# alexrenz/AdaPM

Measured on AMD Instinct MI355X. Metric: pull_push_ops_per_s, higher is better.
Workload: dtype fp32; 1 GPU; model=kge_complex_dim512, entities=10000000, relations=1000, dim=512, neg_samples=16, global_batch=16384, triples=90000000, parallelism=ps-async-dp1, fused_step=True, warmup_extra_steps=400

## Files before the change

### adapm_amd/csrc/core.cpp

```cpp
#include <torch/extension.h>
#include <ATen/Parallel.h>

#include <algorithm>
#include <atomic>
#include <condition_variable>
#include <cstring>
#include <limits>
#include <deque>
#include <map>
#include <queue>
#include <tuple>
#include <memory>
#include <mutex>
#include <random>
#include <thread>
#include <chrono>
#include <unordered_map>
#include <unordered_set>
#include <cstdio>
#include <vector>

#include "common.h"
#include "kernels.h"
#include "ops.h"
// ... 211 lines not shown
    state_ = torch::zeros({USTREAM_STATE_WORDS},
                          torch::TensorOptions().dtype(torch::kInt64).device(dev_));
  }

  static bool supported(int64_t lo, int64_t hi) {
    if (hi <= lo || lo == std::numeric_limits<int64_t>::min()) return false;
    uint64_t span = (uint64_t)hi - (uint64_t)lo;
    return span >= 2 && span <= 0xFFFFFFFFull;
  }

  void import_state(uint64_t state_hi, uint64_t state_lo, uint64_t inc_hi, uint64_t inc_lo,
                    uint64_t has_uint32, uint64_t uinteger) {
    auto h = torch::empty({USTREAM_STATE_WORDS}, torch::kInt64);
    uint64_t* p = reinterpret_cast<uint64_t*>(h.data_ptr<int64_t>());
    p[0] = state_hi, p[1] = state_lo, p[2] = inc_hi, p[3] = inc_lo;
    p[4] = has_uint32 ? 1 : 0, p[5] = uinteger & 0xFFFFFFFFull;
    ustream_build_table(p);
    std::lock_guard<std::mutex> g(mu_);
    adopt(current_stream(dev_));
    state_.copy_(h);
  }

  std::vector<uint64_t> export_state() {
    torch::Tensor h;
    {
      std::lock_guard<std::mutex> g(mu_);
      adopt(current_stream(dev_));
      h = state_.slice(0, 0, USTREAM_GEN_WORDS).cpu();
    }
    const uint64_t* p = reinterpret_cast<const uint64_t*>(h.data_ptr<int64_t>());
    return std::vector<uint64_t>(p, p + USTREAM_GEN_WORDS);
  }

  torch::Tensor draw(int64_t n, int64_t slack = -1) {
    TORCH_CHECK(n >= 0, "UniformStream.draw: n must be >= 0");
    auto opt = torch::TensorOptions().dtype(torch::kInt64).device(dev_);
    auto out = torch::empty({n}, opt);
    if (n == 0) return out;
    if (slack < 0) {
      double p = (double)thr_ / 4294967296.0;
      double w0 = (double)n / (1.0 - p);
      slack = (int64_t)std::ceil(w0 - (double)n + 8.0 * std::sqrt(w0 * p) / (1.0 - p)) + 16;
    }
    const int64_t words = n + slack;
    std::lock_guard<std::mutex> g(mu_);
    void* st = current_stream(dev_);
    adopt(st);
    auto tmp = torch::empty({ustream_tmp_words(words)}, opt);
    uint64_t* sp = reinterpret_cast<uint64_t*>(state_.data_ptr<int64_t>());
    if (dev_.is_cuda()) {
#ifdef ADAPM_WITH_HIP
      uniform_draw_gpu(sp, lo_, excl_, thr_, n, words, out.data_ptr<int64_t>(),
                       tmp.data_ptr<int64_t>(), st);
#else
      TORCH_CHECK(false, "UniformStream: built without HIP");
#endif
    } else {
      uniform_draw_cpu(sp, lo_, excl_, thr_, n, words, out.data_ptr<int64_t>(),
                       tmp.data_ptr<int64_t>());
    }
    return out;
  }

  int64_t lo() const { return lo_; }
  int64_t hi() const { return hi_; }
  const torch::Device& device() const { return dev_; }

 private:
  void adopt(void* st) {
#ifdef ADAPM_WITH_HIP
    if (dev_.is_cuda() && have_owner_ && st != owner_) hipStreamSynchronize((hipStream_t)owner_);
#endif
    owner_ = st;
    have_owner_ = true;
  }

  int64_t lo_, hi_;
  uint32_t excl_ = 0, thr_ = 0;
  torch::Device dev_;
  torch::Tensor state_;
  std::mutex mu_;
  void* owner_ = nullptr;
  bool have_owner_ = false;
};


// ... 2108 lines not shown
      ChannelState& C = channels_[ch];
      C.rounds++;
      if (globally_idle) {
        if (++C.idle_streak >= 2) C.idle2_events++;
      } else {
        C.idle_streak = 0;
      }
    }
    rounds_cv_.notify_all();
  }

  py::dict debug_pending() {
    py::dict d;
    {
      std::lock_guard<std::mutex> g(tickets_mu_);
      d["tickets"] = tickets_.size();
    }
    py::list outq, respq, rounds;
    for (auto& C : channels_) {
      std::lock_guard<std::mutex> g(C.mu);
      outq.append(C.out_queue.size());
      respq.append(C.responses.size());
      rounds.append(C.rounds.load());
    }
    d["out_queues"] = outq;
    d["responses"] = respq;
    d["rounds"] = rounds;
    return d;
  }


  bool fused_plain_ok(void* st) {
    if (clocks_.size() != 1 || fused_multi_stream_) return false;
    if (!fused_marks_.defined()) {
      if (getenv("ADAPM_FUSED_ATOMIC")) {
        fused_multi_stream_ = true;
        return false;
      }
      fused_marks_ = torch::zeros({rowmark_words(num_keys_)},
                                  torch::TensorOptions().dtype(torch::kInt32).device(dev_));
      if (getenv("ADAPM_FUSED_STATS"))
        fused_shared_stat_ =
            torch::zeros({1}, torch::TensorOptions().dtype(torch::kInt64).device(dev_));
      fused_marks_stream_ = st;
      return true;
    }
    if (st == fused_marks_stream_) return true;
#ifdef ADAPM_WITH_HIP
    hipStreamSynchronize((hipStream_t)fused_marks_stream_);
#endif
    fused_multi_stream_ = true;
    return false;
  }

  void check_fused_identity(const char* name, int64_t D) {
    TORCH_CHECK(world_ == 1, name, " requires a single rank (all keys local)");
    TORCH_CHECK(uniform_len_ == 2 * D, name, ": store rows must be [emb|accum] = 2D");
    TORCH_CHECK(layout_identity_.load(), name, " requires the identity layout");
    TORCH_CHECK(dev_.is_cuda(), name, " is the GPU fast path");
  }

  void count_fused_ops(int64_t keys) {
    stat_pull_keys_ += keys;
    stat_pull_local_ += keys;
    stat_push_keys_ += keys;
    stat_push_local_ += keys;
    stat_pulls_ += 1;
    stat_pushes_ += 1;
  }

  struct StagedKeys {
    torch::Tensor dev;
    std::vector<const int64_t*> ptr;
  };
  StagedKeys stage_keys(const char* name, std::initializer_list<const torch::Tensor*> parts) {
    int64_t total = 0;
    for (auto* t : parts) {
      check_keys(*t);
      total += t->numel();
    }
    auto blob = torch::empty(
        {total}, torch::TensorOptions().dtype(torch::kInt64).pinned_memory(true));
    int64_t* dst = blob.data_ptr<int64_t>();
    const uint64_t lim = (uint64_t)num_keys_;
    uint64_t bad = 0;
    for (auto* t : parts) {
      const int64_t* kp = t->data_ptr<int64_t>();
      const int64_t n = t->numel();
      for (int64_t i = 0; i < n; ++i) {
        int64_t k = kp[i];
        dst[i] = k;
        bad |= ((uint64_t)k >= lim);
      }
      dst += n;
    }
    if (bad)
      for (auto* t : parts) check_key_range(*t);
    StagedKeys sk;
    sk.dev = torch::empty({total}, torch::TensorOptions().dtype(torch::kInt64).device(dev_));
#ifdef ADAPM_WITH_HIP
    auto stream = c10::hip::getCurrentHIPStreamMasqueradingAsCUDA(dev_.index());
    TORCH_CHECK(copy_keys_gpu(sk.dev.data_ptr<int64_t>(), blob.data_ptr<int64_t>(), total,
                              (void*)stream.stream()),
                name, ": the pinned key staging buffer is not visible to the device");
    at::getHostAllocator(at::kCUDA)->record_event(
        blob.data_ptr(), blob.storage().data_ptr().get_context(), stream.unwrap());
#else
    TORCH_CHECK(false, name, ": built without HIP");
#endif
    const int64_t* dp = sk.dev.data_ptr<int64_t>();
    for (auto* t : parts) {
      sk.ptr.push_back(dp);
      dp += t->numel();
    }
    return sk;
  }

  std::tuple<torch::Tensor, torch::Tensor> kge_step_fused_impl(
      const torch::Tensor& keys_s, const torch::Tensor& keys_r, const torch::Tensor& keys_o,
      const torch::Tensor* keys_neg, UniformStream* us, int64_t N, int64_t D, double lr,
      double eps) {
    check_fused_identity("kge_step_fused", D);
    check_step_lanes("kge_step_fused", "D/2", D / 2);
    int64_t B = keys_s.numel();
    TORCH_CHECK(keys_r.numel() == B && keys_o.numel() == B);
    StagedKeys sk;
    torch::Tensor drawn;
    const int64_t* kn;
    if (us) {
      TORCH_CHECK(us->lo() >= 0 && us->hi() <= num_keys_, "kge_step_fused_sampled: stream range [",
                  us->lo(), ", ", us->hi(), ") exceeds the store's ", num_keys_, " keys");
      TORCH_CHECK(us->device() == dev_,
                  "kge_step_fused_sampled: stream is not on the store's device");
      TORCH_CHECK(N >= 0 && B * N > 0, "kge_step_fused_sampled: nothing to draw");
      sk = stage_keys("kge_step_fused", {&keys_s, &keys_r, &keys_o});
      drawn = us->draw(B * N);
      kn = drawn.data_ptr<int64_t>();
    } else {
      TORCH_CHECK(keys_neg->numel() == B * N);
      sk = stage_keys("kge_step_fused", {&keys_s, &keys_r, &keys_o, keys_neg});
      kn = sk.ptr[3];
    }
    const int64_t *ks = sk.ptr[0], *kr = sk.ptr[1], *ko = sk.ptr[2];

    auto loss = torch::empty({B}, torch::TensorOptions().dtype(torch::kFloat32).device(dev_));
    void* st = current_stream(dev_);
    {
      InflightGuard g(this);
      std::unique_lock<std::mutex> mg(fused_mu_);
      if (fused_plain_ok(st)) {
        RowMarkKeys mk{{ks, kr, ko, kn}, {B, B, B, B * N}, 4};
        auto* marks = reinterpret_cast<uint32_t*>(fused_marks_.data_ptr<int32_t>());
        rowmark_set_gpu(marks, mk, st);
        kge_complex_step_fused_gpu(
            slab_.data, mk.keys[0], mk.keys[1], mk.keys[2], mk.keys[3], loss.data_ptr<float>(),
            (int)B, (int)N, (int)D, Slab::padded(uniform_len_), world_, (float)lr, (float)eps,
            st, marks,
            fused_shared_stat_.defined()
                ? reinterpret_cast<unsigned long long*>(fused_shared_stat_.data_ptr<int64_t>())
                : nullptr);
        rowmark_clear_gpu(marks, mk, st);
        stat_fused_plain_ += 1;
      } else {
        mg.unlock();
        kge_complex_step_fused_gpu(slab_.data, ks, kr, ko, kn, loss.data_ptr<float>(), (int)B,
                                   (int)N, (int)D, Slab::padded(uniform_len_), world_, (float)lr,
                                   (float)eps, st);
        stat_fused_atomic_ += 1;
      }
    }
    count_fused_ops(3 * B + B * N);
    return {loss, drawn};
  }

  torch::Tensor kge_step_fused(torch::Tensor keys_s, torch::Tensor keys_r, torch::Tensor keys_o,
                               torch::Tensor keys_neg, int64_t N, int64_t D, double lr,
                               double eps) {
    return std::get<0>(
        kge_step_fused_impl(keys_s, keys_r, keys_o, &keys_neg, nullptr, N, D, lr, eps));
  }

  std::tuple<torch::Tensor, torch::Tensor> kge_step_fused_sampled(
      torch::Tensor keys_s, torch::Tensor keys_r, torch::Tensor keys_o, UniformStream& us,
      int64_t N, int64_t D, double lr, double eps) {
    return kge_step_fused_impl(keys_s, keys_r, keys_o, nullptr, &us, N, D, lr, eps);
  }

  struct FusedResolve {
    std::vector<std::vector<int64_t>> offs;
    std::vector<int64_t> missed;
    int64_t b_hit = 0;
    std::vector<const int64_t*> ptr;
    std::vector<torch::Tensor> dev;
  };

  FusedResolve resolve_fused(const std::vector<std::pair<const int64_t*, int>>& arrs,
                             int64_t B) {
    FusedResolve out;
    const int na = (int)arrs.size();
    constexpr int64_t G = 1024;
    int64_t nchunks = (B + G - 1) / G;
    struct Part {
      std::vector<std::vector<int64_t>> offs;
      std::vector<int64_t> missed;
    };
    std::vector<Part> parts(nchunks);
    pass_pool_.run(nchunks, [&](int64_t c0, int64_t c1) {
      for (int64_t c = c0; c < c1; ++c) {
        Part& P = parts[c];
        P.offs.resize(na);
        int64_t e = std::min(B, (c + 1) * G);
        std::vector<int64_t> tmp;
        for (int64_t b = c * G; b < e; ++b) {
          tmp.clear();
          bool ok = true;
          for (int a = 0; a < na && ok; ++a) {
            const int64_t* kp = arrs[a].first;
            int cnt = arrs[a].second;
// ... 585 lines not shown
  std::atomic<int64_t> t_pass_{0}, t_todev_{0}, t_launch_{0}, t_calls_{0}, t_misc_{0};
  std::atomic<int64_t> t_sy_intents_{0}, t_sy_replicas_{0}, t_sy_build_{0}, t_sy_proc_{0},
      t_sy_apply_{0}, n_sy_deltas_{0}, n_sy_proc_recs_{0}, n_sy_apply_recs_{0};
  bool cpp_timing_ = getenv("ADAPM_CPP_TIMING") != nullptr;
 private:
  std::mutex tickets_mu_;
  std::condition_variable tickets_cv_;
  std::unordered_map<int64_t, std::unique_ptr<Ticket>> tickets_;
  std::unordered_map<int64_t, std::string> failed_tickets_;
  std::string failed_reason_;
  std::atomic<bool> failed_flag_{false};
  std::mutex rounds_mu_;
  std::condition_variable rounds_cv_;

  bool locality_stats_ = false;
  std::vector<std::atomic<uint32_t>> key_accesses_, key_local_;
  std::mutex trace_mu_;
  std::unordered_set<Key> traced_keys_;
  bool trace_all_ = false;
  struct TraceEv { double t; Key k; const char* ev; };
  std::vector<TraceEv> trace_;
  std::chrono::steady_clock::time_point t0_ = std::chrono::steady_clock::now();

  std::atomic<int64_t> hop_hist_[9] = {};
  std::atomic<int64_t> stat_replica_records_{0}, stat_replica_payloads_{0};
  std::atomic<int64_t> stat_pulls_{0}, stat_pushes_{0}, stat_pull_keys_{0}, stat_push_keys_{0},
      stat_pull_local_{0}, stat_push_local_{0}, stat_pull_replica_{0}, stat_push_replica_{0},
      stat_remote_pulls_served_{0}, stat_remote_pushes_served_{0}, stat_relocations_{0},
      stat_relocated_in_{0}, stat_replications_{0}, stat_drops_{0}, stat_forwards_{0},
      stat_dropped_records_{0}, stat_delta_overhops_{0}, stat_bytes_sent_{0},
      stat_bytes_recv_{0}, stat_sampling_checks_{0};

  std::mutex fused_mu_;
  torch::Tensor fused_marks_;
  torch::Tensor fused_shared_stat_;
  void* fused_marks_stream_ = nullptr;
  bool fused_multi_stream_ = false;
  std::atomic<int64_t> stat_fused_plain_{0}, stat_fused_atomic_{0};
};


static float* fp(torch::Tensor& t) { return t.data_ptr<float>(); }
static const float* cfp(const torch::Tensor& t) { return t.data_ptr<float>(); }

static void check_f32(const torch::Tensor& t, const char* name) {
  TORCH_CHECK(t.is_contiguous() && t.scalar_type() == torch::kFloat32, name,
              " must be contiguous float32");
}

void kge_complex_step(torch::Tensor s, torch::Tensor r, torch::Tensor o, torch::Tensor neg,
                      torch::Tensor ds, torch::Tensor dr, torch::Tensor do_, torch::Tensor dneg,
                      torch::Tensor loss, int64_t N, int64_t D, double lr, double eps) {
  for (auto* t : {&s, &r, &o, &neg, &ds, &dr, &do_, &dneg, &loss}) check_f32(*t, "kge tensor");
  int B = (int)loss.numel();
  if (s.is_cuda()) {
    TORCH_CHECK(hip_available(), "kge_complex_step: CUDA tensor but no HIP device");
    check_step_lanes("kge_complex_step", "D/2", D / 2);
    kge_complex_step_gpu(cfp(s), cfp(r), cfp(o), cfp(neg), fp(ds), fp(dr), fp(do_), fp(dneg),
                         fp(loss), B, (int)N, (int)D, (float)lr, (float)eps,
                         current_stream(s.device()));
  } else {
    kge_complex_step_cpu(cfp(s), cfp(r), cfp(o), cfp(neg), fp(ds), fp(dr), fp(do_), fp(dneg),
                         fp(loss), B, (int)N, (int)D, (float)lr, (float)eps);
  }
}

void rescal_step(torch::Tensor s, torch::Tensor r, torch::Tensor o, torch::Tensor neg,
                 torch::Tensor ds, torch::Tensor drl, torch::Tensor do_, torch::Tensor dneg,
                 torch::Tensor loss, int64_t N, int64_t D, double lr, double eps) {
// ... 317 lines not shown
      .def(py::init<int64_t, torch::Tensor, int, int, int, int, std::string, double, int, bool,
                    int64_t, int64_t, double>(),
           py::arg("num_keys"), py::arg("value_lengths"), py::arg("rank"), py::arg("world"),
           py::arg("num_channels"), py::arg("num_workers"), py::arg("device"),
           py::arg("capacity_factor") = 2.0, py::arg("techniques") = 0,
           py::arg("location_caches") = true, py::arg("device_cap_floats") = 0,
           py::arg("host_spill_floats") = 0, py::arg("sync_threshold") = 0.0)
      .def("pull", &Server::pull, py::call_guard<py::gil_scoped_release>())
      .def("push", &Server::push, py::call_guard<py::gil_scoped_release>())
      .def("pull_if_local", &Server::pull_if_local, py::call_guard<py::gil_scoped_release>())
      .def("is_local", &Server::is_local)
      .def("intent", &Server::intent, py::call_guard<py::gil_scoped_release>())
      .def("advance_clock", &Server::advance_clock)
      .def("current_clock", &Server::current_clock)
      .def("worker_clocks", &Server::worker_clocks)
      .def("wait", &Server::wait, py::call_guard<py::gil_scoped_release>())
      .def("wait_all", &Server::wait_all, py::call_guard<py::gil_scoped_release>())
      .def("is_finished", &Server::is_finished)
      .def("round_counts", &Server::round_counts)
      .def("wait_rounds", &Server::wait_rounds, py::call_guard<py::gil_scoped_release>())
      .def("idle_counts", &Server::idle_counts)
      .def("wait_idle", &Server::wait_idle, py::call_guard<py::gil_scoped_release>())
      .def("set_intent_ahead", &Server::set_intent_ahead)
      .def("sync_collect", &Server::sync_collect, py::call_guard<py::gil_scoped_release>())
      .def("sync_process", &Server::sync_process, py::call_guard<py::gil_scoped_release>())
      .def("sync_respond", &Server::sync_respond, py::call_guard<py::gil_scoped_release>())
      .def("sync_apply", &Server::sync_apply, py::call_guard<py::gil_scoped_release>())
      .def("sync_finish", &Server::sync_finish, py::arg("ch"),
           py::arg("globally_idle") = false, py::call_guard<py::gil_scoped_release>())
      .def("fail", &Server::fail, py::call_guard<py::gil_scoped_release>())
      .def("failed_reason", &Server::failed_reason)
      .def("scan_local", &Server::scan_local, py::call_guard<py::gil_scoped_release>())
      .def("kge_step_fused", &Server::kge_step_fused, py::call_guard<py::gil_scoped_release>())
      .def("kge_step_fused_sampled", &Server::kge_step_fused_sampled,
           py::call_guard<py::gil_scoped_release>())
      .def("w2v_step_fused", &Server::w2v_step_fused, py::call_guard<py::gil_scoped_release>())
      .def("mf_step_fused", &Server::mf_step_fused, py::call_guard<py::gil_scoped_release>())
      .def("kge_step_fused_general", &Server::kge_step_fused_general,
           py::call_guard<py::gil_scoped_release>())
      .def("w2v_step_fused_general", &Server::w2v_step_fused_general,
           py::call_guard<py::gil_scoped_release>())
      .def("mf_step_fused_general", &Server::mf_step_fused_general,
           py::call_guard<py::gil_scoped_release>())
      .def("rebalance_spill", &Server::rebalance_spill, py::arg("max_moves") = 4096,
           py::call_guard<py::gil_scoped_release>())
      .def("key_tier", &Server::key_tier)
      .def("get_len", &Server::get_len)
      .def("uniform_len", &Server::uniform_len)
      .def("layout_identity", &Server::layout_identity)
      .def("num_keys", &Server::num_keys)
      .def("rank", &Server::rank)
      .def("world", &Server::world)
      .def("num_channels", &Server::num_channels)
      .def("owner_hint", &Server::owner_hint)
      .def("enable_locality_stats", &Server::enable_locality_stats)
      .def("enable_key_trace", &Server::enable_key_trace)
      .def("debug_key_state", &Server::debug_key_state)
      .def("debug_set_loc_cache", &Server::debug_set_loc_cache)
      .def("debug_pending", &Server::debug_pending)
      .def("dump_locality_stats", &Server::dump_locality_stats)
      .def("dump_traces", &Server::dump_traces)
      .def("stats", &Server::stats)
      .def("debug_flags", &Server::debug_flags);
}
```

### adapm_amd/csrc/kernels.h

```cpp
#pragma once
#include <cstdint>

namespace adapm {

constexpr int STEP_MAX_LANES = 8 * 256;

void kge_complex_step_gpu(const float* s, const float* r, const float* o, const float* neg,
                          float* ds, float* dr, float* do_, float* dneg, float* loss,
                          int B, int N, int D, float lr, float eps, void* stream);
void kge_complex_step_cpu(const float* s, const float* r, const float* o, const float* neg,
                          float* ds, float* dr, float* do_, float* dneg, float* loss,
                          int B, int N, int D, float lr, float eps);

struct RowMarkKeys {
  const int64_t* keys[4];
  int64_t n[4];
  int count;
};
inline int64_t rowmark_words(int64_t rows) { return (rows + 15) / 16; }
void rowmark_set_gpu(uint32_t* marks, const RowMarkKeys& ks, void* stream);
void rowmark_clear_gpu(uint32_t* marks, const RowMarkKeys& ks, void* stream);

void kge_complex_step_fused_gpu(float* slab, const int64_t* keys_s, const int64_t* keys_r,
                                const int64_t* keys_o, const int64_t* keys_neg, float* loss,
                                int B, int N, int D, int32_t plen, int world, float lr,
                                float eps, void* stream, const uint32_t* marks = nullptr,
                                unsigned long long* shared_stat = nullptr);

void kge_complex_step_fused_offs_cpu(float* slab, const int64_t* offs_s, const int64_t* offs_r,
                                     const int64_t* offs_o, const int64_t* offs_neg, float* loss,
                                     int B, int N, int D, float lr, float eps);
void w2v_sgns_step_fused_offs_cpu(float* slab, const int64_t* offs_ctr, const int64_t* offs_ctx,
                                  const int64_t* offs_neg, float* loss, int B, int N, int D,
                                  float lr, float eps);
void mf_update_step_fused_offs_cpu(float* slab, const int64_t* offs_w, const int64_t* offs_h,
                                   const float* x, float* loss, int B, int R, float lr,
                                   float lambda, float eps);

void w2v_sgns_step_fused_gpu(float* slab, const int64_t* keys_ctr, const int64_t* keys_ctx,
                             const int64_t* keys_neg, float* loss, int B, int N, int D,
                             int32_t plen, int world, float lr, float eps, void* stream);

void mf_update_step_fused_gpu(float* slab, const int64_t* keys_w, const int64_t* keys_h,
                              const float* x, float* loss, int B, int R, int32_t plen,
                              int world, float lr, float lambda, float eps, void* stream);

void kge_complex_score_gpu(const float* s, const float* r, const float* cand, float* scores,
                           int B, int E, int D, void* stream);
void kge_complex_score_cpu(const float* s, const float* r, const float* cand, float* scores,
                           int B, int E, int D);

void rescal_step_gpu(const float* s, const float* r, const float* o, const float* neg,
                     float* ds, float* drl, float* do_, float* dneg, float* loss, int B, int N,
                     int D, float lr, float eps, void* stream);
void rescal_step_cpu(const float* s, const float* r, const float* o, const float* neg,
                     float* ds, float* drl, float* do_, float* dneg, float* loss, int B, int N,
                     int D, float lr, float eps);

void w2v_sgns_step_gpu(const float* ctr, const float* ctx, const float* neg, float* dctr,
                       float* dctx, float* dneg, float* loss, int B, int N, int D, float lr,
                       float eps, void* stream);
void w2v_sgns_step_cpu(const float* ctr, const float* ctx, const float* neg, float* dctr,
                       float* dctx, float* dneg, float* loss, int B, int N, int D, float lr,
                       float eps);

void mf_update_step_gpu(const float* w, const float* h, const float* x, float* dw, float* dh,
                        float* loss, int B, int R, float lr, float lambda, float eps,
                        void* stream);
void mf_update_step_cpu(const float* w, const float* h, const float* x, float* dw, float* dh,
                        float* loss, int B, int R, float lr, float lambda, float eps);

void mf_loss_gpu(const float* w, const float* h, const float* x, double* acc2, int B, int R,
                 float lambda, void* stream);
void mf_loss_cpu(const float* w, const float* h, const float* x, float* out2, int B, int R,
                 float lambda);

void alias_draw_gpu(const float* prob, const int32_t* alias, int64_t n, uint64_t seed,
                    int64_t N, int64_t* out, void* stream);
void alias_draw_cpu(const float* prob, const int32_t* alias, int64_t n, uint64_t seed,
                    int64_t N, int64_t* out);

void uniform_draw_gpu(uint64_t* state, int64_t lo, uint32_t excl, uint32_t thr, int64_t n,
                      int64_t words, int64_t* out, int64_t* tmp, void* stream);
void uniform_draw_cpu(uint64_t* state, int64_t lo, uint32_t excl, uint32_t thr, int64_t n,
                      int64_t words, int64_t* out, int64_t* tmp);

bool copy_keys_gpu(int64_t* dst, const int64_t* src_host, int64_t n, void* stream);

}

namespace adapm {


void kge_complex_score_mfma_gpu(const float* s, const float* r, const float* cand,
                                float* scores, float* qbuf, int B, int E, int D, void* stream);

void mfma_grouped_gemm_gpu(const float* S, const float* W, const float* R, float* out,
                           const int* starts, int G, int D, int sstride, int wstride,
                           int64_t rstride, int out_rstride, int64_t ostride, int mode,
                           int total_tiles, void* stream);

void rescal_mid_gpu(const float* U, const float* o, const float* neg, float* do_, float* dneg,
                    float* Wm, float* loss, int B, int N, int D, float lr, float eps,
                    void* stream);

void adagrad_rows_gpu(const float* grad, const float* rows, float* out, int64_t n_rows,
                      int dvals, int gstride, int rstride, float lr, float eps, void* stream);

}
```

### adapm_amd/csrc/kernels_hip.hip

```cpp
#include <hip/hip_runtime.h>
#include <algorithm>
#include <type_traits>

#include "kernels.h"
#include "ustream.h"

namespace adapm {

#define KT 256

static inline unsigned grid_for(int64_t n, int64_t cap = 16384) {
  return (unsigned)std::min(std::max<int64_t>(n, 1), cap);
}

static_assert(STEP_MAX_LANES == 8 * KT, "dispatch_kpt stops at KPT = 8");
template <typename F>
static inline void dispatch_kpt(int lanes, F&& f) {
  if (lanes <= KT) f(std::integral_constant<int, 1>{});
  else if (lanes <= 2 * KT) f(std::integral_constant<int, 2>{});
  else if (lanes <= 4 * KT) f(std::integral_constant<int, 4>{});
  else f(std::integral_constant<int, 8>{});
}

__device__ inline float block_reduce_sum(float v, float* lds) {
// ... 283 lines not shown
                           int B, int E, int D, void* stream) {
  hipLaunchKernelGGL(k_kge_score, dim3(grid_for((int64_t)B * E)), dim3(KT), 0,
                     (hipStream_t)stream, s, r, cand, scores, B, E, D);
}
void w2v_sgns_step_gpu(const float* ctr, const float* ctx, const float* neg, float* dctr,
                       float* dctx, float* dneg, float* loss, int B, int N, int D, float lr,
                       float eps, void* stream) {
  dispatch_kpt(D, [&](auto kpt) {
    hipLaunchKernelGGL(k_w2v_step<decltype(kpt)::value>, dim3(grid_for(B)), dim3(KT), 0,
                       (hipStream_t)stream, ctr, ctx, neg, dctr, dctx, dneg, loss, B, N, D, lr,
                       eps);
  });
}
void mf_update_step_gpu(const float* w, const float* h, const float* x, float* dw, float* dh,
                        float* loss, int B, int R, float lr, float lambda, float eps,
                        void* stream) {
  hipLaunchKernelGGL(k_mf_step, dim3(grid_for(B)), dim3(KT), 0, (hipStream_t)stream, w, h, x, dw,
                     dh, loss, B, R, lr, lambda, eps);
}

}

namespace adapm {
void alias_draw_gpu(const float* prob, const int32_t* alias, int64_t n, uint64_t seed,
                    int64_t N, int64_t* out, void* stream) {
  if (N == 0) return;
  hipLaunchKernelGGL(k_alias_draw, dim3(grid_for((N + 255) / 256, 4096)), dim3(256), 0,
                     (hipStream_t)stream, prob, alias, n, seed, N, out);
}
}

namespace adapm {

static_assert(USTREAM_BLOCK == KT, "one chunk per thread of a KT workgroup");

__device__ inline int64_t block_reduce_i64(int64_t v, int64_t* lds) {
  for (int off = 32; off > 0; off >>= 1) v += __shfl_xor(v, off, 64);
  if ((threadIdx.x & 63) == 0) lds[threadIdx.x >> 6] = v;
  __syncthreads();
  int64_t out = 0;
  for (int i = 0; i < KT / 64; ++i) out += lds[i];
  __syncthreads();
  return out;
}

template <typename T>
__device__ inline T* ustream_block_keys(T* tmp, int64_t nb, int64_t block) {
  return tmp + USTREAM_TMP_COUNTS + nb + block * (KT * USTREAM_CHUNK) + threadIdx.x;
}

__global__ void __launch_bounds__(KT)
k_ustream_gen(const uint64_t* __restrict__ state, UStreamRange r, int64_t words, int64_t chunks,
              int64_t* __restrict__ tmp, int64_t nb) {
  __shared__ int64_t lds[KT / 64];
  const int64_t c = (int64_t)blockIdx.x * KT + threadIdx.x;
  int64_t cnt = 0;
  if (c < chunks)
    cnt = ustream_gen_chunk(state, r, words, c, ustream_block_keys(tmp, nb, blockIdx.x), KT);
  cnt = block_reduce_i64(cnt, lds);
  if (threadIdx.x == 0) {
    tmp[USTREAM_TMP_COUNTS + blockIdx.x] = cnt;
  }
}

__global__ void __launch_bounds__(KT)
k_ustream_compact(uint64_t* __restrict__ state, UStreamRange r, int64_t n, int64_t words,
                  int64_t chunks, const int64_t* __restrict__ tmp, int64_t nb,
                  int64_t* __restrict__ out) {
  __shared__ int64_t lds[KT / 64];
  __shared__ int wave_tot[KT / 64];
  const int64_t* counts = tmp + USTREAM_TMP_COUNTS;
  int64_t part = 0;
  for (int64_t i = threadIdx.x; i < (int64_t)blockIdx.x; i += KT) part += counts[i];
  const int64_t off = block_reduce_i64(part, lds);
  const int64_t c = (int64_t)blockIdx.x * KT + threadIdx.x;
  const bool live = off < n && c < chunks;
  const int64_t* kc = ustream_block_keys(tmp, nb, blockIdx.x);
  int64_t k[USTREAM_CHUNK];
  int cnt = 0;
#pragma unroll
  for (int i = 0; i < USTREAM_CHUNK; ++i) {
    k[i] = live ? kc[i * KT] : USTREAM_REJECTED;
    cnt += (k[i] != USTREAM_REJECTED);
  }
  const int lane = threadIdx.x & 63, wave = threadIdx.x >> 6;
  int incl = cnt;
  for (int d = 1; d < 64; d <<= 1) {
    int y = __shfl_up(incl, d, 64);
    if (lane >= d) incl += y;
  }
  if (lane == 63) wave_tot[wave] = incl;
  __syncthreads();
  int64_t idx = off + incl - cnt;
  for (int i = 0; i < wave; ++i) idx += wave_tot[i];
  int64_t consumed = 0;
#pragma unroll
  for (int i = 0; i < USTREAM_CHUNK; ++i) {
    if (k[i] == USTREAM_REJECTED) continue;
    if (idx < n) {
      out[idx] = k[i];
      if (idx == n - 1) consumed = c * USTREAM_CHUNK + i + 1;
    }
    ++idx;
  }
  if (consumed) {
    ustream_finish(state, r, n, words, n, consumed, out);
  } else if (blockIdx.x == nb - 1 && threadIdx.x == 0) {
    int64_t total = off;
    for (int i = 0; i < KT / 64; ++i) total += wave_tot[i];
    if (total < n) ustream_finish(state, r, n, words, total, 0, out);
  }
}

void uniform_draw_gpu(uint64_t* state, int64_t lo, uint32_t excl, uint32_t thr, int64_t n,
                      int64_t words, int64_t* out, int64_t* tmp, void* stream) {
  if (n <= 0) return;
  const UStreamRange r{lo, excl, thr};
  const int64_t chunks = ustream_chunks(words), nb = ustream_blocks(words);
  auto st = (hipStream_t)stream;
  hipLaunchKernelGGL(k_ustream_gen, dim3((unsigned)nb), dim3(KT), 0, st, state, r, words, chunks,
                     tmp, nb);
  hipLaunchKernelGGL(k_ustream_compact, dim3((unsigned)nb), dim3(KT), 0, st, state, r, n, words,
                     chunks, tmp, nb, out);
}

__global__ void k_copy_keys(int64_t* __restrict__ dst, const int64_t* __restrict__ src,
                            int64_t n) {
  int64_t i = (int64_t)blockIdx.x * KT + threadIdx.x;
  if (i < n) dst[i] = src[i];
}

bool copy_keys_gpu(int64_t* dst, const int64_t* src_host, int64_t n, void* stream) {
  if (n <= 0) return true;
  void* src = nullptr;
  if (hipHostGetDevicePointer(&src, const_cast<int64_t*>(src_host), 0) != hipSuccess || !src) {
    (void)hipGetLastError();
    return false;
  }
  hipLaunchKernelGGL(k_copy_keys, dim3((unsigned)((n + KT - 1) / KT)), dim3(KT), 0,
                     (hipStream_t)stream, dst, static_cast<const int64_t*>(src), n);
  return true;
}
}

namespace adapm {

__global__ void k_rescal_step(const float* __restrict__ s, const float* __restrict__ r,
                              const float* __restrict__ o, const float* __restrict__ neg,
                              float* __restrict__ ds, float* __restrict__ drl,
                              float* __restrict__ do_, float* __restrict__ dneg,
                              float* __restrict__ loss, int B, int N, int D, float lr,
                              float eps) {
  extern __shared__ __attribute__((aligned(16))) float smem[];
  float* Rm = smem;
  float* u = Rm + D * D;
  float* w = u + D;
  float* es = w + D;
  float* red = es + D;
  const int erow = 2 * D;
  const int64_t rrow = 2LL * D * D;

  for (int b = blockIdx.x; b < B; b += gridDim.x) {
    const float* sb = s + (int64_t)b * erow;
    const float* rb = r + (int64_t)b * rrow;
    for (int i = threadIdx.x; i < D * D; i += KT) Rm[i] = rb[i];
    for (int i = threadIdx.x; i < D; i += KT) {
      es[i] = sb[i];
      w[i] = 0.f;
    }
    __syncthreads();
    for (int j = threadIdx.x; j < D; j += KT) {
      float a = 0.f;
      for (int i = 0; i < D; ++i) a += Rm[i * D + j] * es[i];
// ... 24 lines not shown
    float* dsb = ds + (int64_t)b * erow;
    for (int i = threadIdx.x; i < D; i += KT) {
      float a = 0.f;
      for (int k = 0; k < D; ++k) a += Rm[i * D + k] * w[k];
      write_delta(&dsb[i], &dsb[D + i], a, sb[D + i], lr, eps);
    }
    float* drb = drl + (int64_t)b * rrow;
    for (int idx = threadIdx.x; idx < D * D; idx += KT) {
      int i = idx / D, k = idx % D;
      const int64_t acc = (int64_t)D * D + idx;
      write_delta(&drb[idx], &drb[acc], es[i] * w[k], rb[acc], lr, eps);
    }
    __syncthreads();
  }
}

void rescal_step_gpu(const float* s, const float* r, const float* o, const float* neg,
                     float* ds, float* drl, float* do_, float* dneg, float* loss, int B, int N,
                     int D, float lr, float eps, void* stream) {
  size_t smem = (size_t)(D * D + 3 * D + KT / 64) * sizeof(float);
  if (B < 1) return;
  hipLaunchKernelGGL(k_rescal_step, dim3(grid_for(B, 8192)), dim3(KT), smem, (hipStream_t)stream,
                     s, r, o, neg, ds, drl, do_, dneg, loss, B, N, D, lr, eps);
}

}

namespace adapm {

__device__ inline float* row_at(float* slab, int64_t v, int32_t plen, int world) {
  return world ? slab + (v / world) * (int64_t)plen : slab + v;
}

__device__ inline uint32_t* rowmark_word(uint32_t* marks, int64_t row) { return marks + (row >> 4); }
__device__ inline int rowmark_shift(int64_t row) { return 2 * (int)(row & 15); }

__device__ inline int64_t rowmark_key(const RowMarkKeys& ks, int64_t i) {
  int a = 0;
  while (a < ks.count - 1 && i >= ks.n[a]) {
    i -= ks.n[a];
    ++a;
  }
  return ks.keys[a][i];
}

__global__ void k_rowmark_set(uint32_t* __restrict__ marks, RowMarkKeys ks, int64_t total) {
  int64_t i = (int64_t)blockIdx.x * blockDim.x + threadIdx.x;
  if (i >= total) return;
  int64_t row = rowmark_key(ks, i);
  uint32_t bit = 1u << rowmark_shift(row);
  uint32_t old = atomicOr(rowmark_word(marks, row), bit);
  if ((old & bit) && !(old & (bit << 1))) atomicOr(rowmark_word(marks, row), bit << 1);
}

__global__ void k_rowmark_clear(uint32_t* __restrict__ marks, RowMarkKeys ks, int64_t total) {
  int64_t i = (int64_t)blockIdx.x * blockDim.x + threadIdx.x;
  if (i >= total) return;
  *rowmark_word(marks, rowmark_key(ks, i)) = 0u;
}

void rowmark_set_gpu(uint32_t* marks, const RowMarkKeys& ks, void* stream) {
  int64_t total = 0;
  for (int a = 0; a < ks.count; ++a) total += ks.n[a];
  if (total == 0) return;
  hipLaunchKernelGGL(k_rowmark_set, dim3((unsigned)((total + KT - 1) / KT)), dim3(KT), 0,
                     (hipStream_t)stream, marks, ks, total);
}

void rowmark_clear_gpu(uint32_t* marks, const RowMarkKeys& ks, void* stream) {
  int64_t total = 0;
  for (int a = 0; a < ks.count; ++a) total += ks.n[a];
  if (total == 0) return;
  hipLaunchKernelGGL(k_rowmark_clear, dim3((unsigned)((total + KT - 1) / KT)), dim3(KT), 0,
                     (hipStream_t)stream, marks, ks, total);
}

template <bool UNIQ>
__device__ inline bool row_shared(const uint32_t* __restrict__ marks, int64_t key) {
  if (!UNIQ) return true;
  return (marks[key >> 4] >> (rowmark_shift(key) + 1)) & 1u;
}

__device__ inline float plain_add(float a, float delta) {
#pragma clang fp contract(off)
  return a + delta;
}

__device__ inline void slab_adagrad(float* p_emb, float* p_acc, float g, float emb, float acc,
                                    float lr, float eps, bool shared) {
  float d = adagrad_delta(g, acc, lr, eps);
  if (shared) {
    atomicAdd(p_emb, d);
    atomicAdd(p_acc, g * g);
  } else {
    *p_emb = plain_add(emb, d);
    *p_acc = plain_add(acc, g * g);
  }
}

#define SLAB_ADAGRAD_COMPLEX(row, shared, g_re, g_im, emb_re, emb_im, acc_re, acc_im) \
  do {                                                                                \
    float G_re = (acc_re) + (g_re) * (g_re);                                          \
    float G_im = (acc_im) + (g_im) * (g_im);                                          \
    float d_re = -lr * (g_re) * __frsqrt_rn(G_re + eps);                              \
    float d_im = -lr * (g_im) * __frsqrt_rn(G_im + eps);                              \
    if (shared) {                                                                     \
      atomicAdd(&(row)[k], d_re);                                                     \
      atomicAdd(&(row)[dc + k], d_im);                                                \
      atomicAdd(&(row)[D + k], (g_re) * (g_re));                                      \
      atomicAdd(&(row)[D + dc + k], (g_im) * (g_im));                                 \
    } else {                                                                          \
      (row)[k] = plain_add(emb_re, d_re);                                             \
      (row)[dc + k] = plain_add(emb_im, d_im);                                        \
      (row)[D + k] = plain_add(acc_re, (g_re) * (g_re));                              \
      (row)[D + dc + k] = plain_add(acc_im, (g_im) * (g_im));                         \
    }                                                                                 \
  } while (0)

template <int KPT, bool UNIQ>
__global__ void k_kge_step_fused(float* __restrict__ slab, const int64_t* __restrict__ keys_s,
                                 const int64_t* __restrict__ keys_r,
                                 const int64_t* __restrict__ keys_o,
                                 const int64_t* __restrict__ keys_neg, float* __restrict__ loss,
                                 int B, int N, int D, int32_t plen, int world, float lr,
                                 float eps, const uint32_t* __restrict__ marks,
                                 unsigned long long* __restrict__ shared_stat) {
  __shared__ float lds[KT / 64];
  const int dc = D >> 1;
  const int w = UNIQ ? 1 : world;
  for (int b = blockIdx.x; b < B; b += gridDim.x) {
    const int64_t key_s = keys_s[b], key_r = keys_r[b];
    const float* sb = row_at(slab, key_s, plen, w);
    const float* rb = row_at(slab, key_r, plen, w);
    const bool s_shared = row_shared<UNIQ>(marks, key_s);
    const bool r_shared = row_shared<UNIQ>(marks, key_r);
    unsigned n_shared = (unsigned)s_shared + (unsigned)r_shared;

    float s_re[KPT], s_im[KPT], r_re[KPT], r_im[KPT];
    float a_sre[KPT], a_sim[KPT], a_rre[KPT], a_rim[KPT];
    float u_re[KPT], u_im[KPT];
#pragma unroll
    for (int i = 0; i < KPT; ++i) {
      int k = threadIdx.x + i * KT;
      a_sre[i] = a_sim[i] = a_rre[i] = a_rim[i] = 0.f;
      if (k < dc) {
        s_re[i] = sb[k];
        s_im[i] = sb[dc + k];
        r_re[i] = rb[k];
        r_im[i] = rb[dc + k];
        u_re[i] = s_re[i] * r_re[i] - s_im[i] * r_im[i];
        u_im[i] = s_im[i] * r_re[i] + s_re[i] * r_im[i];
      } else {
        s_re[i] = s_im[i] = r_re[i] = r_im[i] = u_re[i] = u_im[i] = 0.f;
      }
    }

    float lsum = 0.f;
    for (int j = 0; j <= N; ++j) {
      int64_t ok = (j == 0) ? keys_o[b] : keys_neg[(int64_t)b * N + (j - 1)];
      float* ob = row_at(slab, ok, plen, w);
      const bool o_shared = row_shared<UNIQ>(marks, ok);
      n_shared += (unsigned)o_shared;
      float y = (j == 0) ? 1.f : -1.f;
      float part = 0.f;
      float o_re[KPT], o_im[KPT], Go_re[KPT], Go_im[KPT];
#pragma unroll
      for (int i = 0; i < KPT; ++i) {
        int k = threadIdx.x + i * KT;
        o_re[i] = k < dc ? ob[k] : 0.f;
        o_im[i] = k < dc ? ob[dc + k] : 0.f;
        Go_re[i] = k < dc ? ob[D + k] : 0.f;
        Go_im[i] = k < dc ? ob[D + dc + k] : 0.f;
        part += u_re[i] * o_re[i] + u_im[i] * o_im[i];
      }
      float psi = block_reduce_sum(part, lds);
      float c = -y * sigmoidf(-y * psi);
      if (threadIdx.x == 0) lsum += softplusf(-y * psi);

#pragma unroll
      for (int i = 0; i < KPT; ++i) {
        int k = threadIdx.x + i * KT;
        if (k >= dc) continue;
        a_sre[i] += c * (r_re[i] * o_re[i] + r_im[i] * o_im[i]);
        a_sim[i] += c * (r_re[i] * o_im[i] - r_im[i] * o_re[i]);
        a_rre[i] += c * (s_re[i] * o_re[i] + s_im[i] * o_im[i]);
        a_rim[i] += c * (s_re[i] * o_im[i] - s_im[i] * o_re[i]);
        float g_re = c * u_re[i];
        float g_im = c * u_im[i];
        SLAB_ADAGRAD_COMPLEX(ob, o_shared, g_re, g_im, o_re[i], o_im[i], Go_re[i], Go_im[i]);
      }
    }
    float* dsb = const_cast<float*>(sb);
    float* drb = const_cast<float*>(rb);
#pragma unroll
    for (int i = 0; i < KPT; ++i) {
      int k = threadIdx.x + i * KT;
      if (k >= dc) continue;
      float Gs_re = sb[D + k], Gs_im = sb[D + dc + k];
      SLAB_ADAGRAD_COMPLEX(dsb, s_shared, a_sre[i], a_sim[i], s_re[i], s_im[i], Gs_re, Gs_im);
      float Gr_re = rb[D + k], Gr_im = rb[D + dc + k];
      SLAB_ADAGRAD_COMPLEX(drb, r_shared, a_rre[i], a_rim[i], r_re[i], r_im[i], Gr_re, Gr_im);
    }
    if (threadIdx.x == 0) {
      loss[b] = lsum;
      if (UNIQ && shared_stat) atomicAdd(shared_stat, (unsigned long long)n_shared);
    }
  }
}

#undef SLAB_ADAGRAD_COMPLEX

void kge_complex_step_fused_gpu(float* slab, const int64_t* keys_s, const int64_t* keys_r,
                                const int64_t* keys_o, const int64_t* keys_neg, float* loss,
                                int B, int N, int D, int32_t plen, int world, float lr,
                                float eps, void* stream, const uint32_t* marks,
                                unsigned long long* shared_stat) {
  if (B < 1) return;
  const bool uniq = marks != nullptr && world == 1;
  if (!uniq) marks = nullptr, shared_stat = nullptr;
  dispatch_kpt(D >> 1, [&](auto kpt) {
    constexpr int KPT = decltype(kpt)::value;
    hipLaunchKernelGGL((uniq ? k_kge_step_fused<KPT, true> : k_kge_step_fused<KPT, false>),
                       dim3(grid_for(B)), dim3(KT), 0, (hipStream_t)stream, slab, keys_s, keys_r,
                       keys_o, keys_neg, loss, B, N, D, plen, world, lr, eps, marks,
                       shared_stat);
  });
}

}

namespace adapm {

template <int KPT>
__global__ void k_w2v_step_fused(float* __restrict__ slab, const int64_t* __restrict__ keys_ctr,
                                 const int64_t* __restrict__ keys_ctx,
                                 const int64_t* __restrict__ keys_neg, float* __restrict__ loss,
                                 int B, int N, int D, int32_t plen, int world, float lr,
                                 float eps) {
  __shared__ float lds[KT / 64];
  for (int b = blockIdx.x; b < B; b += gridDim.x) {
    float* cb = row_at(slab, keys_ctr[b], plen, world);
    float c_emb[KPT], a_c[KPT];
#pragma unroll
    for (int i = 0; i < KPT; ++i) {
      int k = threadIdx.x + i * KT;
      c_emb[i] = k < D ? cb[k] : 0.f;
      a_c[i] = 0.f;
    }
    float lsum = 0.f;
    for (int j = 0; j <= N; ++j) {
      int64_t xk = (j == 0) ? keys_ctx[b] : keys_neg[(int64_t)b * N + (j - 1)];
      float* xb = row_at(slab, xk, plen, world);
      float y = (j == 0) ? 1.f : -1.f;
      float part = 0.f;
      float x_emb[KPT];
#pragma unroll
      for (int i = 0; i < KPT; ++i) {
        int k = threadIdx.x + i * KT;
// ... 68 lines not shown
```

Before: 1.229 billion key-ops/s.

## Replace row-mark bitmap with per-slot owner table claimed during key staging

Duplicate-row detection used to run in separate passes: an atomic set kernel over a packed 2-bit bitmap, then a clear kernel after the step. Now the key copy and uniform-draw compaction kernels write each key's slot index into a per-row owner array (non-atomic, last writer wins). A single resolve kernel then flags both the slots that lost and the winning slot as shared, and the step kernel looks up sharedness by slot index instead of by row. This removes the clear pass and the atomics, and fuses the marking into kernels that already run. In exchange it allocates a full num_keys int32 owner table plus a per-batch shared array, and it relies on the last-writer-wins race to give a consistent winner within each step.

```diff
diff --git a/adapm_amd/csrc/core.cpp b/adapm_amd/csrc/core.cpp
--- a/adapm_amd/csrc/core.cpp
+++ b/adapm_amd/csrc/core.cpp
@@ -267,8 +267,11 @@
     return std::vector<uint64_t>(p, p + USTREAM_GEN_WORDS);
   }
 
-  torch::Tensor draw(int64_t n, int64_t slack = -1) {
+  torch::Tensor draw(int64_t n, int64_t slack = -1) { return draw_owned(n, slack, RowOwners{}, 0); }
+
+  torch::Tensor draw_owned(int64_t n, int64_t slack, RowOwners own, int64_t first) {
     TORCH_CHECK(n >= 0, "UniformStream.draw: n must be >= 0");
+    TORCH_CHECK(!own.owner || dev_.is_cuda(), "UniformStream: row owners need a device stream");
     auto opt = torch::TensorOptions().dtype(torch::kInt64).device(dev_);
     auto out = torch::empty({n}, opt);
     if (n == 0) return out;
@@ -286,7 +289,7 @@
     if (dev_.is_cuda()) {
 #ifdef ADAPM_WITH_HIP
       uniform_draw_gpu(sp, lo_, excl_, thr_, n, words, out.data_ptr<int64_t>(),
-                       tmp.data_ptr<int64_t>(), st);
+                       tmp.data_ptr<int64_t>(), st, own, first);
 #else
       TORCH_CHECK(false, "UniformStream: built without HIP");
 #endif
@@ -2461,22 +2464,22 @@
 
   bool fused_plain_ok(void* st) {
     if (clocks_.size() != 1 || fused_multi_stream_) return false;
-    if (!fused_marks_.defined()) {
+    if (!fused_owner_.defined()) {
       if (getenv("ADAPM_FUSED_ATOMIC")) {
         fused_multi_stream_ = true;
         return false;
       }
-      fused_marks_ = torch::zeros({rowmark_words(num_keys_)},
+      fused_owner_ = torch::zeros({num_keys_},
                                   torch::TensorOptions().dtype(torch::kInt32).device(dev_));
       if (getenv("ADAPM_FUSED_STATS"))
         fused_shared_stat_ =
             torch::zeros({1}, torch::TensorOptions().dtype(torch::kInt64).device(dev_));
-      fused_marks_stream_ = st;
+      fused_owner_stream_ = st;
       return true;
     }
-    if (st == fused_marks_stream_) return true;
+    if (st == fused_owner_stream_) return true;
 #ifdef ADAPM_WITH_HIP
-    hipStreamSynchronize((hipStream_t)fused_marks_stream_);
+    hipStreamSynchronize((hipStream_t)fused_owner_stream_);
 #endif
     fused_multi_stream_ = true;
     return false;
@@ -2502,7 +2505,8 @@
     torch::Tensor dev;
     std::vector<const int64_t*> ptr;
   };
-  StagedKeys stage_keys(const char* name, std::initializer_list<const torch::Tensor*> parts) {
+  StagedKeys stage_keys(const char* name, std::initializer_list<const torch::Tensor*> parts,
+                        RowOwners own = RowOwners{}) {
     int64_t total = 0;
     for (auto* t : parts) {
       check_keys(*t);
@@ -2530,7 +2534,7 @@
 #ifdef ADAPM_WITH_HIP
     auto stream = c10::hip::getCurrentHIPStreamMasqueradingAsCUDA(dev_.index());
     TORCH_CHECK(copy_keys_gpu(sk.dev.data_ptr<int64_t>(), blob.data_ptr<int64_t>(), total,
-                              (void*)stream.stream()),
+                              (void*)stream.stream(), own),
                 name, ": the pinned key staging buffer is not visible to the device");
     at::getHostAllocator(at::kCUDA)->record_event(
         blob.data_ptr(), blob.storage().data_ptr().get_context(), stream.unwrap());
@@ -2547,56 +2551,58 @@
 
   std::tuple<torch::Tensor, torch::Tensor> kge_step_fused_impl(
       const torch::Tensor& keys_s, const torch::Tensor& keys_r, const torch::Tensor& keys_o,
-      const torch::Tensor* keys_neg, UniformStream* us, int64_t N, int64_t D, double lr,
-      double eps) {
+      const torch::Tensor* keys_neg, UniformStream* us, int64_t us_slack, int64_t N, int64_t D,
+      double lr, double eps) {
     check_fused_identity("kge_step_fused", D);
     check_step_lanes("kge_step_fused", "D/2", D / 2);
     int64_t B = keys_s.numel();
     TORCH_CHECK(keys_r.numel() == B && keys_o.numel() == B);
-    StagedKeys sk;
-    torch::Tensor drawn;
-    const int64_t* kn;
     if (us) {
       TORCH_CHECK(us->lo() >= 0 && us->hi() <= num_keys_, "kge_step_fused_sampled: stream range [",
                   us->lo(), ", ", us->hi(), ") exceeds the store's ", num_keys_, " keys");
       TORCH_CHECK(us->device() == dev_,
                   "kge_step_fused_sampled: stream is not on the store's device");
       TORCH_CHECK(N >= 0 && B * N > 0, "kge_step_fused_sampled: nothing to draw");
-      sk = stage_keys("kge_step_fused", {&keys_s, &keys_r, &keys_o});
-      drawn = us->draw(B * N);
-      kn = drawn.data_ptr<int64_t>();
     } else {
       TORCH_CHECK(keys_neg->numel() == B * N);
-      sk = stage_keys("kge_step_fused", {&keys_s, &keys_r, &keys_o, keys_neg});
-      kn = sk.ptr[3];
-    }
-    const int64_t *ks = sk.ptr[0], *kr = sk.ptr[1], *ko = sk.ptr[2];
-
+    }
     auto loss = torch::empty({B}, torch::TensorOptions().dtype(torch::kFloat32).device(dev_));
     void* st = current_stream(dev_);
+    StagedKeys sk;
+    torch::Tensor drawn;
     {
       InflightGuard g(this);
       std::unique_lock<std::mutex> mg(fused_mu_);
-      if (fused_plain_ok(st)) {
-        RowMarkKeys mk{{ks, kr, ko, kn}, {B, B, B, B * N}, 4};
-        auto* marks = reinterpret_cast<uint32_t*>(fused_marks_.data_ptr<int32_t>());
-        rowmark_set_gpu(marks, mk, st);
-        kge_complex_step_fused_gpu(
-            slab_.data, mk.keys[0], mk.keys[1], mk.keys[2], mk.keys[3], loss.data_ptr<float>(),
-            (int)B, (int)N, (int)D, Slab::padded(uniform_len_), world_, (float)lr, (float)eps,
-            st, marks,
-            fused_shared_stat_.defined()
-                ? reinterpret_cast<unsigned long long*>(fused_shared_stat_.data_ptr<int64_t>())
-                : nullptr);
-        rowmark_clear_gpu(marks, mk, st);
-        stat_fused_plain_ += 1;
+      const bool plain = fused_plain_ok(st);
+      if (!plain) mg.unlock();
+      RowOwners own;
+      torch::Tensor shared;
+      if (plain) {
+        TORCH_CHECK(3 * B + B * N < (int64_t)1 << 31, "kge_step_fused: too many keys in a batch");
+        shared = torch::empty({3 * B + B * N},
+                              torch::TensorOptions().dtype(torch::kInt32).device(dev_));
+        own.owner = fused_owner_.data_ptr<int32_t>();
+        own.shared = reinterpret_cast<uint32_t*>(shared.data_ptr<int32_t>());
+      }
+      const int64_t* kn;
+      if (us) {
+        sk = stage_keys("kge_step_fused", {&keys_s, &keys_r, &keys_o}, own);
+        drawn = us->draw_owned(B * N, us_slack, own, 3 * B);
+        kn = drawn.data_ptr<int64_t>();
       } else {
-        mg.unlock();
-        kge_complex_step_fused_gpu(slab_.data, ks, kr, ko, kn, loss.data_ptr<float>(), (int)B,
-                                   (int)N, (int)D, Slab::padded(uniform_len_), world_, (float)lr,
-                                   (float)eps, st);
-        stat_fused_atomic_ += 1;
-      }
+        sk = stage_keys("kge_step_fused", {&keys_s, &keys_r, &keys_o, keys_neg}, own);
+        kn = sk.ptr[3];
+      }
+      if (plain)
+        rowowner_resolve_gpu(own, RowMarkKeys{{sk.ptr[0], sk.ptr[1], sk.ptr[2], kn},
+                                              {B, B, B, B * N}, 4}, st);
+      kge_complex_step_fused_gpu(
+          slab_.data, sk.ptr[0], sk.ptr[1], sk.ptr[2], kn, loss.data_ptr<float>(), (int)B,
+          (int)N, (int)D, Slab::padded(uniform_len_), world_, (float)lr, (float)eps, st, own,
+          plain && fused_shared_stat_.defined()
+              ? reinterpret_cast<unsigned long long*>(fused_shared_stat_.data_ptr<int64_t>())
+              : nullptr);
+      (plain ? stat_fused_plain_ : stat_fused_atomic_) += 1;
     }
     count_fused_ops(3 * B + B * N);
     return {loss, drawn};
@@ -2606,13 +2612,13 @@
                                torch::Tensor keys_neg, int64_t N, int64_t D, double lr,
                                double eps) {
     return std::get<0>(
-        kge_step_fused_impl(keys_s, keys_r, keys_o, &keys_neg, nullptr, N, D, lr, eps));
+        kge_step_fused_impl(keys_s, keys_r, keys_o, &keys_neg, nullptr, -1, N, D, lr, eps));
   }
 
   std::tuple<torch::Tensor, torch::Tensor> kge_step_fused_sampled(
       torch::Tensor keys_s, torch::Tensor keys_r, torch::Tensor keys_o, UniformStream& us,
-      int64_t N, int64_t D, double lr, double eps) {
-    return kge_step_fused_impl(keys_s, keys_r, keys_o, nullptr, &us, N, D, lr, eps);
+      int64_t N, int64_t D, double lr, double eps, int64_t slack) {
+    return kge_step_fused_impl(keys_s, keys_r, keys_o, nullptr, &us, slack, N, D, lr, eps);
   }
 
   struct FusedResolve {
@@ -3264,9 +3270,9 @@
       stat_bytes_recv_{0}, stat_sampling_checks_{0};
 
   std::mutex fused_mu_;
-  torch::Tensor fused_marks_;
+  torch::Tensor fused_owner_;
   torch::Tensor fused_shared_stat_;
-  void* fused_marks_stream_ = nullptr;
+  void* fused_owner_stream_ = nullptr;
   bool fused_multi_stream_ = false;
   std::atomic<int64_t> stat_fused_plain_{0}, stat_fused_atomic_{0};
 };
@@ -3650,7 +3656,9 @@
       .def("failed_reason", &Server::failed_reason)
       .def("scan_local", &Server::scan_local, py::call_guard<py::gil_scoped_release>())
       .def("kge_step_fused", &Server::kge_step_fused, py::call_guard<py::gil_scoped_release>())
-      .def("kge_step_fused_sampled", &Server::kge_step_fused_sampled,
+      .def("kge_step_fused_sampled", &Server::kge_step_fused_sampled, py::arg("keys_s"),
+           py::arg("keys_r"), py::arg("keys_o"), py::arg("us"), py::arg("N"), py::arg("D"),
+           py::arg("lr"), py::arg("eps"), py::arg("slack") = -1,
            py::call_guard<py::gil_scoped_release>())
       .def("w2v_step_fused", &Server::w2v_step_fused, py::call_guard<py::gil_scoped_release>())
       .def("mf_step_fused", &Server::mf_step_fused, py::call_guard<py::gil_scoped_release>())
diff --git a/adapm_amd/csrc/kernels.h b/adapm_amd/csrc/kernels.h
--- a/adapm_amd/csrc/kernels.h
+++ b/adapm_amd/csrc/kernels.h
@@ -17,14 +17,16 @@
   int64_t n[4];
   int count;
 };
-inline int64_t rowmark_words(int64_t rows) { return (rows + 15) / 16; }
-void rowmark_set_gpu(uint32_t* marks, const RowMarkKeys& ks, void* stream);
-void rowmark_clear_gpu(uint32_t* marks, const RowMarkKeys& ks, void* stream);
+struct RowOwners {
+  int32_t* owner = nullptr;
+  uint32_t* shared = nullptr;
+};
+void rowowner_resolve_gpu(const RowOwners& own, const RowMarkKeys& ks, void* stream);
 
 void kge_complex_step_fused_gpu(float* slab, const int64_t* keys_s, const int64_t* keys_r,
                                 const int64_t* keys_o, const int64_t* keys_neg, float* loss,
                                 int B, int N, int D, int32_t plen, int world, float lr,
-                                float eps, void* stream, const uint32_t* marks = nullptr,
+                                float eps, void* stream, const RowOwners& own = RowOwners{},
                                 unsigned long long* shared_stat = nullptr);
 
 void kge_complex_step_fused_offs_cpu(float* slab, const int64_t* offs_s, const int64_t* offs_r,
@@ -81,11 +83,13 @@
                     int64_t N, int64_t* out);
 
 void uniform_draw_gpu(uint64_t* state, int64_t lo, uint32_t excl, uint32_t thr, int64_t n,
-                      int64_t words, int64_t* out, int64_t* tmp, void* stream);
+                      int64_t words, int64_t* out, int64_t* tmp, void* stream,
+                      RowOwners own = RowOwners{}, int64_t first = 0);
 void uniform_draw_cpu(uint64_t* state, int64_t lo, uint32_t excl, uint32_t thr, int64_t n,
                       int64_t words, int64_t* out, int64_t* tmp);
 
-bool copy_keys_gpu(int64_t* dst, const int64_t* src_host, int64_t n, void* stream);
+bool copy_keys_gpu(int64_t* dst, const int64_t* src_host, int64_t n, void* stream,
+                   RowOwners own = RowOwners{});
 
 }
 
diff --git a/adapm_amd/csrc/kernels_hip.hip b/adapm_amd/csrc/kernels_hip.hip
--- a/adapm_amd/csrc/kernels_hip.hip
+++ b/adapm_amd/csrc/kernels_hip.hip
@@ -339,6 +339,11 @@
 
 namespace adapm {
 
+__device__ inline void rowowner_claim(const RowOwners& w, int64_t row, int64_t me) {
+  w.owner[row] = (int32_t)me;
+  w.shared[me] = 0;
+}
+
 static_assert(USTREAM_BLOCK == KT, "one chunk per thread of a KT workgroup");
 
 __device__ inline int64_t block_reduce_i64(int64_t v, int64_t* lds) {
@@ -373,7 +378,7 @@
 __global__ void __launch_bounds__(KT)
 k_ustream_compact(uint64_t* __restrict__ state, UStreamRange r, int64_t n, int64_t words,
                   int64_t chunks, const int64_t* __restrict__ tmp, int64_t nb,
-                  int64_t* __restrict__ out) {
+                  int64_t* __restrict__ out, RowOwners own, int64_t first) {
   __shared__ int64_t lds[KT / 64];
   __shared__ int wave_tot[KT / 64];
   const int64_t* counts = tmp + USTREAM_TMP_COUNTS;
@@ -406,6 +411,7 @@
     if (k[i] == USTREAM_REJECTED) continue;
     if (idx < n) {
       out[idx] = k[i];
+      if (own.owner) rowowner_claim(own, k[i], first + idx);
       if (idx == n - 1) consumed = c * USTREAM_CHUNK + i + 1;
     }
     ++idx;
@@ -415,12 +421,17 @@
   } else if (blockIdx.x == nb - 1 && threadIdx.x == 0) {
     int64_t total = off;
     for (int i = 0; i < KT / 64; ++i) total += wave_tot[i];
-    if (total < n) ustream_finish(state, r, n, words, total, 0, out);
+    if (total < n) {
+      ustream_finish(state, r, n, words, total, 0, out);
+      if (own.owner)
+        for (int64_t i = total; i < n; ++i) rowowner_claim(own, out[i], first + i);
+    }
   }
 }
 
 void uniform_draw_gpu(uint64_t* state, int64_t lo, uint32_t excl, uint32_t thr, int64_t n,
-                      int64_t words, int64_t* out, int64_t* tmp, void* stream) {
+                      int64_t words, int64_t* out, int64_t* tmp, void* stream, RowOwners own,
+                      int64_t first) {
   if (n <= 0) return;
   const UStreamRange r{lo, excl, thr};
   const int64_t chunks = ustream_chunks(words), nb = ustream_blocks(words);
@@ -428,16 +439,20 @@
   hipLaunchKernelGGL(k_ustream_gen, dim3((unsigned)nb), dim3(KT), 0, st, state, r, words, chunks,
                      tmp, nb);
   hipLaunchKernelGGL(k_ustream_compact, dim3((unsigned)nb), dim3(KT), 0, st, state, r, n, words,
-                     chunks, tmp, nb, out);
+                     chunks, tmp, nb, out, own, first);
 }
 
 __global__ void k_copy_keys(int64_t* __restrict__ dst, const int64_t* __restrict__ src,
-                            int64_t n) {
+                            int64_t n, RowOwners own) {
   int64_t i = (int64_t)blockIdx.x * KT + threadIdx.x;
-  if (i < n) dst[i] = src[i];
-}
-
-bool copy_keys_gpu(int64_t* dst, const int64_t* src_host, int64_t n, void* stream) {
+  if (i >= n) return;
+  const int64_t k = src[i];
+  dst[i] = k;
+  if (own.owner) rowowner_claim(own, k, i);
+}
+
+bool copy_keys_gpu(int64_t* dst, const int64_t* src_host, int64_t n, void* stream,
+                   RowOwners own) {
   if (n <= 0) return true;
   void* src = nullptr;
   if (hipHostGetDevicePointer(&src, const_cast<int64_t*>(src_host), 0) != hipSuccess || !src) {
@@ -445,7 +460,7 @@
     return false;
   }
   hipLaunchKernelGGL(k_copy_keys, dim3((unsigned)((n + KT - 1) / KT)), dim3(KT), 0,
-                     (hipStream_t)stream, dst, static_cast<const int64_t*>(src), n);
+                     (hipStream_t)stream, dst, static_cast<const int64_t*>(src), n, own);
   return true;
 }
 }
@@ -536,9 +551,6 @@
   return world ? slab + (v / world) * (int64_t)plen : slab + v;
 }
 
-__device__ inline uint32_t* rowmark_word(uint32_t* marks, int64_t row) { return marks + (row >> 4); }
-__device__ inline int rowmark_shift(int64_t row) { return 2 * (int)(row & 15); }
-
 __device__ inline int64_t rowmark_key(const RowMarkKeys& ks, int64_t i) {
   int a = 0;
   while (a < ks.count - 1 && i >= ks.n[a]) {
@@ -548,41 +560,25 @@
   return ks.keys[a][i];
 }
 
-__global__ void k_rowmark_set(uint32_t* __restrict__ marks, RowMarkKeys ks, int64_t total) {
+__global__ void k_rowowner_resolve(RowOwners own, RowMarkKeys ks, int64_t total) {
   int64_t i = (int64_t)blockIdx.x * blockDim.x + threadIdx.x;
   if (i >= total) return;
-  int64_t row = rowmark_key(ks, i);
-  uint32_t bit = 1u << rowmark_shift(row);
-  uint32_t old = atomicOr(rowmark_word(marks, row), bit);
-  if ((old & bit) && !(old & (bit << 1))) atomicOr(rowmark_word(marks, row), bit << 1);
-}
-
-__global__ void k_rowmark_clear(uint32_t* __restrict__ marks, RowMarkKeys ks, int64_t total) {
-  int64_t i = (int64_t)blockIdx.x * blockDim.x + threadIdx.x;
-  if (i >= total) return;
-  *rowmark_word(marks, rowmark_key(ks, i)) = 0u;
-}
-
-void rowmark_set_gpu(uint32_t* marks, const RowMarkKeys& ks, void* stream) {
+  const int32_t winner = own.owner[rowmark_key(ks, i)];
+  if (winner != (int32_t)i) own.shared[i] = own.shared[winner] = 1;
+}
+
+void rowowner_resolve_gpu(const RowOwners& own, const RowMarkKeys& ks, void* stream) {
   int64_t total = 0;
   for (int a = 0; a < ks.count; ++a) total += ks.n[a];
   if (total == 0) return;
-  hipLaunchKernelGGL(k_rowmark_set, dim3((unsigned)((total + KT - 1) / KT)), dim3(KT), 0,
-                     (hipStream_t)stream, marks, ks, total);
-}
-
-void rowmark_clear_gpu(uint32_t* marks, const RowMarkKeys& ks, void* stream) {
-  int64_t total = 0;
-  for (int a = 0; a < ks.count; ++a) total += ks.n[a];
-  if (total == 0) return;
-  hipLaunchKernelGGL(k_rowmark_clear, dim3((unsigned)((total + KT - 1) / KT)), dim3(KT), 0,
-                     (hipStream_t)stream, marks, ks, total);
+  hipLaunchKernelGGL(k_rowowner_resolve, dim3((unsigned)((total + KT - 1) / KT)), dim3(KT), 0,
+                     (hipStream_t)stream, own, ks, total);
 }
 
 template <bool UNIQ>
-__device__ inline bool row_shared(const uint32_t* __restrict__ marks, int64_t key) {
+__device__ inline bool row_shared(const uint32_t* __restrict__ shared, int64_t me) {
   if (!UNIQ) return true;
-  return (marks[key >> 4] >> (rowmark_shift(key) + 1)) & 1u;
+  return shared[me] != 0;
 }
 
 __device__ inline float plain_add(float a, float delta) {
@@ -627,7 +623,7 @@
                                  const int64_t* __restrict__ keys_o,
                                  const int64_t* __restrict__ keys_neg, float* __restrict__ loss,
                                  int B, int N, int D, int32_t plen, int world, float lr,
-                                 float eps, const uint32_t* __restrict__ marks,
+                                 float eps, const uint32_t* __restrict__ shared,
                                  unsigned long long* __restrict__ shared_stat) {
   __shared__ float lds[KT / 64];
   const int dc = D >> 1;
@@ -636,8 +632,8 @@
     const int64_t key_s = keys_s[b], key_r = keys_r[b];
     const float* sb = row_at(slab, key_s, plen, w);
     const float* rb = row_at(slab, key_r, plen, w);
-    const bool s_shared = row_shared<UNIQ>(marks, key_s);
-    const bool r_shared = row_shared<UNIQ>(marks, key_r);
+    const bool s_shared = row_shared<UNIQ>(shared, b);
+    const bool r_shared = row_shared<UNIQ>(shared, (int64_t)B + b);
     unsigned n_shared = (unsigned)s_shared + (unsigned)r_shared;
 
     float s_re[KPT], s_im[KPT], r_re[KPT], r_im[KPT];
@@ -663,7 +659,8 @@
     for (int j = 0; j <= N; ++j) {
       int64_t ok = (j == 0) ? keys_o[b] : keys_neg[(int64_t)b * N + (j - 1)];
       float* ob = row_at(slab, ok, plen, w);
-      const bool o_shared = row_shared<UNIQ>(marks, ok);
+      const bool o_shared = row_shared<UNIQ>(
+          shared, (j == 0) ? 2 * (int64_t)B + b : 3 * (int64_t)B + (int64_t)b * N + (j - 1));
       n_shared += (unsigned)o_shared;
       float y = (j == 0) ? 1.f : -1.f;
       float part = 0.f;
@@ -717,17 +714,17 @@
 void kge_complex_step_fused_gpu(float* slab, const int64_t* keys_s, const int64_t* keys_r,
                                 const int64_t* keys_o, const int64_t* keys_neg, float* loss,
                                 int B, int N, int D, int32_t plen, int world, float lr,
-                                float eps, void* stream, const uint32_t* marks,
+                                float eps, void* stream, const RowOwners& own,
                                 unsigned long long* shared_stat) {
   if (B < 1) return;
-  const bool uniq = marks != nullptr && world == 1;
-  if (!uniq) marks = nullptr, shared_stat = nullptr;
+  const bool uniq = own.owner != nullptr && world == 1;
+  if (!uniq) shared_stat = nullptr;
   dispatch_kpt(D >> 1, [&](auto kpt) {
     constexpr int KPT = decltype(kpt)::value;
     hipLaunchKernelGGL((uniq ? k_kge_step_fused<KPT, true> : k_kge_step_fused<KPT, false>),
                        dim3(grid_for(B)), dim3(KT), 0, (hipStream_t)stream, slab, keys_s, keys_r,
-                       keys_o, keys_neg, loss, B, N, D, plen, world, lr, eps, marks,
-                       shared_stat);
+                       keys_o, keys_neg, loss, B, N, D, plen, world, lr, eps,
+                       uniq ? own.shared : nullptr, shared_stat);
   });
 }
 
```

After: 1.130 billion key-ops/s. 8.0% lower.
